# facebookresearch/rela

Measured on AMD Instinct MI355X. Metric: env-steps/s (Ape-X Atari 84x84x4, actor tick + learner grad-step), higher is better.
Workload: dtype f32 (f32 operands as 3 exact bf16 parts on bf16 MFMA; f32-accurate); 1 GPU; Ape-X DQN 80x80 envs/GPU, actor+learner on one MI355X, replay 2^20, B=512, A=18, n=3; device-resident static frames; parallelism=single

## Files before the change

rela_amd/csrc/gemm_s3.h:

```cpp
#pragma once
#include <hip/hip_runtime.h>

#include <algorithm>
#include <type_traits>

#include "common.h"
#include "gemm_f32emu.h"

namespace rela_amd {
namespace s3 {

using f32emu::bf16x2;
using f32emu::bf16x8;
using f32emu::f32x2;
using f32emu::f32x4;
using f32emu::kMaxBlocks;
using f32emu::kStageU4;
using f32emu::TN;
using f32emu::u32x4;
using f32emu::WRegs;

struct ProbConv2 {
  static constexpr int KS = 16, NCG = 1, OC = 64, PS = 64, REC = 192;
  __device__ static uint32_t row_base(int m) {
    const int n = m / 81, pos = m - n * 81;
    const int oy = pos / 9, ox = pos - oy * 9;
    return (uint32_t)(((n * 20 + 2 * oy) * 20 + 2 * ox) * REC);
  }
  __device__ static uint32_t koff(int ks) {
    const int tp = f32emu::ProbConv2::tap(ks);
    return (uint32_t)(((tp >> 2) * 20 + (tp & 3)) * REC);
  }
};
struct ProbConv3 {
  static constexpr int KS = 18, NCG = 1, OC = 64, PS = 128, REC = 384;
  __device__ static uint32_t row_base(int m) {
    const int n = m / 49, pos = m - n * 49;
    const int oy = pos / 7, ox = pos - oy * 7;
    return (uint32_t)(((n * 9 + oy) * 9 + ox) * REC);
  }
  __device__ static uint32_t koff(int ks) {
    const int tp = f32emu::ProbConv3::tap(ks);
    return (uint32_t)(((tp / 3) * 9 + tp % 3) * REC + (ks & 1) * 64);
  }
  __device__ static uint32_t pair_off(int kp) { return koff(2 * kp); }
};
template <int OC_>
struct ProbFcT {
  static constexpr int KS = 98, NCG = OC_ / 64, OC = OC_, PS = 128, REC = 384;
  __device__ static uint32_t row_base(int m) { return (uint32_t)m * (49u * REC); }
  __device__ static uint32_t koff(int ks) { return (uint32_t)((ks >> 1) * REC + (ks & 1) * 64); }
  __device__ static uint32_t pair_off(int kp) { return (uint32_t)(kp * REC); }
};
using ProbFc = ProbFcT<512>;

__device__ __forceinline__ void split3_4(const f32x4& v, uint2& p0, uint2& p1, uint2& p2) {
  const f32x2 a = {v[0], v[1]}, b = {v[2], v[3]};
  const bf16x2 a0 = __builtin_convertvector(a, bf16x2), b0 = __builtin_convertvector(b, bf16x2);
  const f32x2 ra = a - __builtin_convertvector(a0, f32x2), rb = b - __builtin_convertvector(b0, f32x2);
  const bf16x2 a1 = __builtin_convertvector(ra, bf16x2), b1 = __builtin_convertvector(rb, bf16x2);
  const f32x2 sa = ra - __builtin_convertvector(a1, f32x2), sb = rb - __builtin_convertvector(b1, f32x2);
  const bf16x2 a2 = __builtin_convertvector(sa, bf16x2), b2 = __builtin_convertvector(sb, bf16x2);
  p0 = make_uint2(__builtin_bit_cast(uint32_t, a0), __builtin_bit_cast(uint32_t, b0));
  p1 = make_uint2(__builtin_bit_cast(uint32_t, a1), __builtin_bit_cast(uint32_t, b1));
  p2 = make_uint2(__builtin_bit_cast(uint32_t, a2), __builtin_bit_cast(uint32_t, b2));
}

constexpr int kGemmT = 512;
constexpr int kGemmWaves = kGemmT / 64;
constexpr int kBlockCols = 128;
constexpr int TMV = 7;
constexpr int CT = 1;
static_assert(kGemmWaves * CT * 16 == kBlockCols, "the waves of a block tile its columns");
constexpr int kABuf = TMV * 6144;
constexpr int kBSlot = CT * 3072;
constexpr int kLdsB = 2 * kABuf;
constexpr int kLdsSpare = kLdsB + kGemmWaves * 2 * kBSlot;
constexpr int kLdsTotal = kLdsSpare + 1024;
static_assert(kLdsTotal <= 160 * 1024, "LDS budget");
__host__ __device__ constexpr int glds_per_wave(int nt) { return (6 * nt + kGemmWaves - 1) / kGemmWaves; }

typedef __attribute__((address_space(3))) uint8_t* lds_ptr_t;
typedef const __attribute__((address_space(1))) uint8_t* gbl_ptr_t;
__device__ __forceinline__ void glds16(const uint8_t* g, uint8_t* l) {
  __builtin_amdgcn_global_load_lds((gbl_ptr_t)g, (lds_ptr_t)l, 16, 0, 0);
}
#ifndef S3_GEMM_ABLATE
#define S3_GEMM_ABLATE 0
#endif
#ifndef S3_GEMM_AHEAD
#define S3_GEMM_AHEAD 1
#endif
constexpr int kAheadTiles = S3_GEMM_AHEAD;
template <int OFF>
__device__ __forceinline__ u32x4 lds_read128(uint32_t addr) {
  u32x4 r;
  asm volatile("ds_read_b128 %0, %1 offset:%2" : "=v"(r) : "v"(addr), "n"(OFF) : "memory");
  return r;
}
template <int N>
__device__ __forceinline__ void wait_lgkm(u32x4& a, u32x4& b, u32x4& c) {
  asm volatile("s_waitcnt lgkmcnt(%3)" : "+v"(a), "+v"(b), "+v"(c) : "n"(N) : "memory");
}
template <int N>
__device__ __forceinline__ void wait_vm() {
  asm volatile("s_waitcnt vmcnt(%0)" ::"n"(N) : "memory");
}
template <int I>
using IC = std::integral_constant<int, I>;
template <int N, class F>
__device__ __forceinline__ void static_for(F&& f) {
  if constexpr (N > 0) {
    static_for<N - 1>(f);
    f(IC<N - 1>{});
  }
}

struct Pipe {
  uint32_t g;
  uint32_t s;
};

template <class P>
__device__ __forceinline__ void issue_weights(const uint8_t* wsrc, uint8_t* lds, uint32_t bring, int k, uint32_t slot, uint32_t lane) {
  const uint8_t* src = wsrc + (size_t)k * (kStageU4 * 16) + lane * 16;
  uint8_t* dst = lds + bring + slot * kBSlot;
  if constexpr (S3_GEMM_ABLATE == 2) return;
#pragma unroll
  for (int q = 0; q < CT * 3; ++q) glds16(src + q * 1024, dst + q * 1024);
}

template <class P, int NT, int J>
__device__ __forceinline__ void k_pass(const uint8_t* __restrict__ Xb, const uint8_t* __restrict__ wsrc, uint8_t* lds, uint32_t lds0,
                                       const uint32_t (&offc)[J], const uint32_t (&offn)[J], const uint32_t (&ldst)[J],
                                       uint32_t frag_base, uint32_t wave, f32x4 (&acc)[NT][CT], f32x4 (&accs)[NT][CT], Pipe& pp,
                                       int kp0, int kp1) {
  constexpr int WL = 3 * CT;
  const uint32_t lane = threadIdx.x & 63;
  const uint32_t bring = kLdsB + wave * 2 * kBSlot;
  for (int kp = kp0; kp < kp1; ++kp) {
    const uint32_t abuf = (pp.g & 1) * kABuf;
    wait_vm<WL>();
    __builtin_amdgcn_s_barrier();
    {
      int k1 = 2 * kp + 1;
      issue_weights<P>(wsrc, lds, bring, k1, (pp.s + 1) & 1, lane);
      int k2 = kp + 1;
      const bool nextp = k2 >= kp1;
      if (nextp) k2 = kp0;
      const uint8_t* src = Xb + P::pair_off(k2);
      const uint32_t dst = ((pp.g + 1) & 1) * kABuf;
      if constexpr (S3_GEMM_ABLATE != 1) {
#pragma unroll
        for (int j = 0; j < J; ++j)
          glds16(src + (nextp ? offn[j] : offc[j]), lds + (ldst[j] >= (uint32_t)kLdsSpare ? ldst[j] : dst + ldst[j]));
      }
    }
    static_for<2>([&](auto hh) {
      constexpr int H = decltype(hh)::value;
      if constexpr (H == 1) {
        int k2 = 2 * kp + 2;
        if (k2 >= 2 * kp1) k2 = 2 * kp0;
        issue_weights<P>(wsrc, lds, bring, k2, (pp.s + 1) & 1, lane);
      }
      wait_vm<J + WL>();
      const uint32_t wa = lds0 + bring + (pp.s & 1) * kBSlot + lane * 16;
      u32x4 wq[CT][3];
      static_for<CT>([&](auto jj) {
        constexpr int JJ = decltype(jj)::value;
        wq[JJ][0] = lds_read128<JJ * 3072>(wa);
        wq[JJ][1] = lds_read128<JJ * 3072 + 1024>(wa);
        wq[JJ][2] = lds_read128<JJ * 3072 + 2048>(wa);
      });
      const uint32_t xa = lds0 + abuf + frag_base + H * 512;
      constexpr int RING = kAheadTiles + 1, PRE = NT < kAheadTiles ? NT : kAheadTiles;
      u32x4 x[RING][3];
      static_for<PRE>([&](auto tt) {
        constexpr int T = decltype(tt)::value;
        x[T][0] = lds_read128<T * 6144>(xa);
        x[T][1] = lds_read128<T * 6144 + 2048>(xa);
        x[T][2] = lds_read128<T * 6144 + 4096>(xa);
      });
      constexpr int AHEAD = PRE * 3;
      static_for<CT>([&](auto jj) {
        constexpr int JJ = decltype(jj)::value;
        wait_lgkm<AHEAD + 3 * (CT - 1 - JJ)>(wq[JJ][0], wq[JJ][1], wq[JJ][2]);
      });
      bf16x8 wf[CT][3];
#pragma unroll
      for (int j = 0; j < CT; ++j)
#pragma unroll
        for (int q = 0; q < 3; ++q) wf[j][q] = __builtin_bit_cast(bf16x8, wq[j][q]);
      static_for<NT>([&](auto tt) {
        constexpr int T = decltype(tt)::value;
        constexpr int C = T % RING;
        if constexpr (T + kAheadTiles < NT) {
          constexpr int N2 = (T + kAheadTiles) % RING;
          x[N2][0] = lds_read128<(T + kAheadTiles) * 6144>(xa);
          x[N2][1] = lds_read128<(T + kAheadTiles) * 6144 + 2048>(xa);
          x[N2][2] = lds_read128<(T + kAheadTiles) * 6144 + 4096>(xa);
        }
        constexpr int YOUNGER = 3 * ((T + kAheadTiles < NT ? T + kAheadTiles : NT - 1) - T);
        wait_lgkm<YOUNGER>(x[C][0], x[C][1], x[C][2]);
        const bf16x8 x0 = __builtin_bit_cast(bf16x8, x[C][0]), x1 = __builtin_bit_cast(bf16x8, x[C][1]),
                     x2 = __builtin_bit_cast(bf16x8, x[C][2]);
#pragma unroll
        for (int j = 0; j < CT; ++j) {
          accs[T][j] = __builtin_amdgcn_mfma_f32_16x16x32_bf16(wf[j][2], x0, accs[T][j], 0, 0, 0);
          accs[T][j] = __builtin_amdgcn_mfma_f32_16x16x32_bf16(wf[j][0], x2, accs[T][j], 0, 0, 0);
          accs[T][j] = __builtin_amdgcn_mfma_f32_16x16x32_bf16(wf[j][1], x1, accs[T][j], 0, 0, 0);
          accs[T][j] = __builtin_amdgcn_mfma_f32_16x16x32_bf16(wf[j][1], x0, accs[T][j], 0, 0, 0);
          accs[T][j] = __builtin_amdgcn_mfma_f32_16x16x32_bf16(wf[j][0], x1, accs[T][j], 0, 0, 0);
          acc[T][j] = __builtin_amdgcn_mfma_f32_16x16x32_bf16(wf[j][0], x0, acc[T][j], 0, 0, 0);
        }
        __builtin_amdgcn_sched_barrier(0);
      });
      pp.s += 1;
    });
    pp.g += 1;
  }
}

enum { kEpiRelu = 0, kEpiReluS3 = 1, kEpiRaw = 2, kEpiBias = 3 };
template <class P, int EPI>
__global__ __launch_bounds__(kGemmT, 1) void gemm_s3(const uint8_t* __restrict__ Xb, const uint4* __restrict__ Wp,
                                                 const float* __restrict__ bias, void* __restrict__ out_, int M) {
  constexpr int NCG = P::OC / kBlockCols;
  constexpr bool OUT_S3 = EPI == kEpiReluS3;
  const int kp0 = (int)((P::KS / 2) * blockIdx.y / gridDim.y), kp1 = (int)((P::KS / 2) * (blockIdx.y + 1) / gridDim.y);
  static_assert(P::OC % kBlockCols == 0, "a block owns 128 columns");
  __shared__ __attribute__((aligned(1024))) uint8_t lds[kLdsTotal];
  const uint32_t lds0 = (uint32_t)(size_t)(lds_ptr_t)lds;
  const int tid = threadIdx.x, lane = tid & 63, li = lane & 15, g = lane >> 4;
  const int wave = __builtin_amdgcn_readfirstlane(tid >> 6);
  const int xcd = blockIdx.x & 7, bi = blockIdx.x >> 3;
  const int cg = bi % NCG;
  const int rb = (bi / NCG) * 8 + xcd;
  const int nrb = gridDim.x / NCG;
  const int rt_total = (M + 15) >> 4;
  const int r0 = (int)((int64_t)rt_total * rb / nrb), r1 = (int)((int64_t)rt_total * (rb + 1) / nrb);
  const int cnt = r1 - r0;
  if (cnt <= 0) return;
  const int passes = (cnt + TMV - 1) / TMV;
  const int base = cnt / passes, rem = cnt - base * passes;
  const int ntmax = base + (rem ? 1 : 0);
  auto first_of = [&](int p) { return p < rem ? (base + 1) * p : (base + 1) * rem + base * (p - rem); };
  auto size_of = [&](int p) { return p < rem ? base + 1 : base; };
  const int cg64 = cg * 2 + (wave >> 2), u0 = wave & 3;
  const uint8_t* wsrc = reinterpret_cast<const uint8_t*>(Wp) + ((size_t)cg64 * P::KS * kStageU4 + (size_t)u0 * 3 * 64) * 16;
  const int col0 = cg * kBlockCols + 16 * CT * wave + 4 * g;
  const uint32_t frag_base = (uint32_t)((li >> 3) * 1024 + (16 * (g >> 1) + 2 * (li & 7) + (g & 1)) * 16);
  const int lr = (lane & 15) >> 1, lu = 2 * (lane >> 4) + (lane & 1);

  f32x4 bv[CT];
#pragma unroll
  for (int j = 0; j < CT; ++j) {
    if constexpr (EPI == kEpiRaw)
      bv[j] = f32x4{0.f, 0.f, 0.f, 0.f};
    else
      bv[j] = *reinterpret_cast<const f32x4*>(bias + col0 + 16 * j);
    asm volatile("" : "+v"(bv[j]));
  }
  Pipe pp{0u, 0u};

  auto run = [&](auto ntm) {
    constexpr int NTM = decltype(ntm)::value, J = glds_per_wave(NTM);
    uint32_t offc[J], offn[J], ldst[J];
    auto set_off = [&](uint32_t (&off)[J], int p) {
      const int nt = size_of(p), t0 = r0 + first_of(p);
#pragma unroll
      for (int j = 0; j < J; ++j) {
        int i = wave + kGemmWaves * j;
        if (i >= 6 * nt) i = 0;
        const int part = (i >> 1) % 3, t = i / 6, b = i & 1;
        const int row = min((t0 + t) * 16 + b * 8 + lr, M - 1);
        off[j] = P::row_base(row) + (uint32_t)(part * 128 + lu * 16);
      }
    };
#pragma unroll
    for (int j = 0; j < J; ++j) {
      const int i = wave + kGemmWaves * j;
      ldst[j] = i < 6 * ntmax ? (uint32_t)i * 1024u : (uint32_t)kLdsSpare;
    }
    set_off(offc, 0);
    set_off(offn, min(1, passes - 1));
    {
      const uint8_t* src = Xb + P::pair_off(kp0);
#pragma unroll
      for (int j = 0; j < J; ++j) glds16(src + offc[j], lds + ldst[j]);
      issue_weights<P>(wsrc, lds, kLdsB + wave * 2 * kBSlot, 2 * kp0, 0, lane);
    }
    auto one_pass = [&](auto ntag, int p) {
      constexpr int NT = decltype(ntag)::value;
      f32x4 acc[NT][CT], accs[NT][CT];
#pragma unroll
      for (int t = 0; t < NT; ++t)
#pragma unroll
        for (int j = 0; j < CT; ++j) acc[t][j] = bv[j], accs[t][j] = f32x4{0.f, 0.f, 0.f, 0.f};
      k_pass<P, NT, J>(Xb, wsrc, lds, lds0, offc, offn, ldst, frag_base, wave, acc, accs, pp, kp0, kp1);
      const int t0 = r0 + first_of(p);
#pragma unroll
      for (int t = 0; t < NT; ++t) {
        const int row = (t0 + t) * 16 + li;
        if (row < M) {
#pragma unroll
          for (int j = 0; j < CT; ++j) {
            f32x4 v = acc[t][j] + accs[t][j];
            if constexpr (EPI == kEpiRelu || EPI == kEpiReluS3) {
#pragma unroll
              for (int r = 0; r < 4; ++r) v[r] = v[r] > 0.f ? v[r] : 0.f;
            }
            if constexpr (OUT_S3) {
              uint8_t* o = reinterpret_cast<uint8_t*>(out_) + (size_t)row * (6 * P::OC) + (col0 + 16 * j) * 2;
              uint2 p0, p1, p2;
              split3_4(v, p0, p1, p2);
              *reinterpret_cast<uint2*>(o) = p0;
              *reinterpret_cast<uint2*>(o + 2 * P::OC) = p1;
              *reinterpret_cast<uint2*>(o + 4 * P::OC) = p2;
            } else {
              *reinterpret_cast<f32x4*>(reinterpret_cast<float*>(out_) + ((size_t)blockIdx.y * M + row) * P::OC + col0 + 16 * j) = v;
            }
          }
        }
      }
    };
    for (int p = 0; p < passes; ++p) {
      if (size_of(p) == NTM)
        one_pass(IC<NTM>{}, p);
      else if constexpr (NTM > 1)
        one_pass(IC<NTM - 1>{}, p);
#pragma unroll
      for (int j = 0; j < J; ++j) offc[j] = offn[j];
      set_off(offn, min(p + 2, passes - 1));
    }
  };
  switch (ntmax) {
    case 1: run(IC<1>{}); break;
    case 2: run(IC<2>{}); break;
    case 3: run(IC<3>{}); break;
    case 4: run(IC<4>{}); break;
    case 5: run(IC<5>{}); break;
    case 6: run(IC<6>{}); break;
    default: run(IC<7>{}); break;
  }
  wait_vm<0>();
}

struct Plan {
  int nrb, slices;
};
template <class P>
inline Plan plan(int M, bool may_split) {
  constexpr int NCG = P::OC / kBlockCols;
  const int rt_total = (M + 15) / 16;
  const int full = kMaxBlocks / 2;
  Plan pl;
  pl.nrb = (std::min(full / NCG, rt_total) + 7) / 8 * 8;
  pl.slices = 1;
  if (may_split && pl.nrb * NCG * 4 <= full * 3) {
    pl.nrb = ((rt_total + 3) / 4 + 7) / 8 * 8;
    pl.slices = std::max(1, std::min(8, full / (pl.nrb * NCG)));
  }
  return pl;
}
template <class P, int EPI>
inline void launch(const void* X, const uint4* Wp, const float* bias, void* out, int M, hipStream_t s, Plan pl) {
  constexpr int NCG = P::OC / kBlockCols;
  hipLaunchKernelGGL((gemm_s3<P, EPI>), dim3(pl.nrb * NCG, EPI == kEpiRaw ? pl.slices : 1), dim3(kGemmT), 0, s,
                     reinterpret_cast<const uint8_t*>(X), Wp, bias, out, M);
}
template <class P, int EPI>
inline void launch(const void* X, const uint4* Wp, const float* bias, void* out, int M, hipStream_t s) {
  launch<P, EPI>(X, Wp, bias, out, M, s, plan<P>(M, false));
}

template <int C>
__global__ void split_s3(const float* __restrict__ x, uint8_t* __restrict__ rec, int64_t pixels) {
  const int64_t i = (int64_t)blockIdx.x * blockDim.x + threadIdx.x;
  if (i >= pixels * (C / 4)) return;
  const int64_t px = i / (C / 4);
  const int c4 = (int)(i - px * (C / 4));
  const f32x4 v = *reinterpret_cast<const f32x4*>(x + px * C + c4 * 4);
  uint2 p0, p1, p2;
  split3_4(v, p0, p1, p2);
  uint8_t* o = rec + px * (6 * C) + c4 * 8;
  *reinterpret_cast<uint2*>(o) = p0;
  *reinterpret_cast<uint2*>(o + 2 * C) = p1;
  *reinterpret_cast<uint2*>(o + 4 * C) = p2;
}
template <int C>
__global__ void unsplit_s3(const uint8_t* __restrict__ rec, float* __restrict__ x, int64_t pixels) {
  const int64_t i = (int64_t)blockIdx.x * blockDim.x + threadIdx.x;
  if (i >= pixels * (C / 4)) return;
  const int64_t px = i / (C / 4);
  const int c4 = (int)(i - px * (C / 4));
  const uint8_t* r = rec + px * (6 * C) + c4 * 8;
  const uint2 p0 = *reinterpret_cast<const uint2*>(r), p1 = *reinterpret_cast<const uint2*>(r + 2 * C),
              p2 = *reinterpret_cast<const uint2*>(r + 4 * C);
  auto f = [](uint32_t w, int hi) { return __builtin_bit_cast(float, hi ? (w & 0xffff0000u) : (w << 16)); };
  f32x4 v;
  v[0] = (f(p0.x, 0) + f(p1.x, 0)) + f(p2.x, 0);
  v[1] = (f(p0.x, 1) + f(p1.x, 1)) + f(p2.x, 1);
  v[2] = (f(p0.y, 0) + f(p1.y, 0)) + f(p2.y, 0);
  v[3] = (f(p0.y, 1) + f(p1.y, 1)) + f(p2.y, 1);
  *reinterpret_cast<f32x4*>(x + px * C + c4 * 4) = v;
}

}
}
```

Before: 3.694 million env-steps/s.

## Interleave LDS-DMA issues across MFMA slots via compile-time pair schedule

```diff
diff --git a/rela_amd/csrc/gemm_s3.h b/rela_amd/csrc/gemm_s3.h
--- a/rela_amd/csrc/gemm_s3.h
+++ b/rela_amd/csrc/gemm_s3.h
@@ -130,40 +130,98 @@
   for (int q = 0; q < CT * 3; ++q) glds16(src + q * 1024, dst + q * 1024);
 }
 
-template <class P, int NT, int J>
+#ifndef S3_GEMM_PLACE
+#define S3_GEMM_PLACE 0
+#endif
+#ifndef S3_GEMM_PLACE_HI
+#define S3_GEMM_PLACE_HI S3_GEMM_PLACE
+#endif
+#ifndef S3_GEMM_PRIO
+#define S3_GEMM_PRIO 0
+#endif
+constexpr int kMaxGldsRun = 2;
+template <int NT, int J, int PL>
+struct PairSched {
+  static constexpr int JA = S3_GEMM_ABLATE == 1 ? 0 : J;
+  static constexpr int WL = S3_GEMM_ABLATE == 2 ? 0 : 3 * CT;
+  static constexpr int N = JA + 2 * WL;
+  static constexpr int SUB = N > 2 * NT ? 2 : 1;
+  static constexpr int S = 2 * NT * SUB;
+  static constexpr int CAP = N > S ? (N + S - 1) / S : 1;
+  static constexpr int pos(int i) {
+    int p = PL == 0 ? i / CAP : PL == 1 ? i * S / N : S - 1 - (N - 1 - i) / CAP;
+    if (i >= JA + WL) {
+      const int lo = S / 2 + (i - JA - WL) / CAP;
+      if (p < lo) p = lo;
+    }
+    return p;
+  }
+  static constexpr int count_at(int p) {
+    int c = 0;
+    for (int i = 0; i < N; ++i) c += pos(i) == p;
+    return c;
+  }
+  static constexpr int first_half() {
+    int c = 0;
+    for (int i = 0; i < N; ++i) c += pos(i) < S / 2;
+    return c;
+  }
+  static constexpr bool valid() {
+    for (int i = 0; i < N; ++i) {
+      if (pos(i) < 0 || pos(i) >= S) return false;
+      if (i && pos(i) < pos(i - 1)) return false;
+      if (i >= JA + WL && pos(i) < S / 2) return false;
+    }
+    for (int p = 0; p < S; ++p)
+      if (count_at(p) > kMaxGldsRun) return false;
+    if (S3_GEMM_ABLATE == 0 && first_half() == 0) return false;
+    return true;
+  }
+  static_assert(valid(), "the pair's LDS-DMA schedule");
+};
+
+template <class P, int NT, int J, int PL>
 __device__ __forceinline__ void k_pass(const uint8_t* __restrict__ Xb, const uint8_t* __restrict__ wsrc, uint8_t* lds, uint32_t lds0,
                                        const uint32_t (&offc)[J], const uint32_t (&offn)[J], const uint32_t (&ldst)[J],
                                        uint32_t frag_base, uint32_t wave, f32x4 (&acc)[NT][CT], f32x4 (&accs)[NT][CT], Pipe& pp,
                                        int kp0, int kp1) {
-  constexpr int WL = 3 * CT;
+  using SC = PairSched<NT, J, PL>;
+  static_assert(CT == 1, "the positions of PairSched are those of one column tile's MFMAs");
   const uint32_t lane = threadIdx.x & 63;
   const uint32_t bring = kLdsB + wave * 2 * kBSlot;
   for (int kp = kp0; kp < kp1; ++kp) {
     const uint32_t abuf = (pp.g & 1) * kABuf;
-    wait_vm<WL>();
+    wait_vm<2 * SC::WL>();
     __builtin_amdgcn_s_barrier();
-    {
-      int k1 = 2 * kp + 1;
-      issue_weights<P>(wsrc, lds, bring, k1, (pp.s + 1) & 1, lane);
-      int k2 = kp + 1;
-      const bool nextp = k2 >= kp1;
-      if (nextp) k2 = kp0;
-      const uint8_t* src = Xb + P::pair_off(k2);
-      const uint32_t dst = ((pp.g + 1) & 1) * kABuf;
-      if constexpr (S3_GEMM_ABLATE != 1) {
-#pragma unroll
-        for (int j = 0; j < J; ++j)
-          glds16(src + (nextp ? offn[j] : offc[j]), lds + (ldst[j] >= (uint32_t)kLdsSpare ? ldst[j] : dst + ldst[j]));
+    int k2 = kp + 1;
+    const bool nextp = k2 >= kp1;
+    if (nextp) k2 = kp0;
+    const uint8_t* asrc = Xb + P::pair_off(k2);
+    const uint32_t adst = ((pp.g + 1) & 1) * kABuf;
+    const uint8_t* wsrc2 = wsrc + (size_t)(2 * k2) * (kStageU4 * 16) + lane * 16;
+    uint8_t* const wdst0 = lds + bring + (pp.s & 1) * kBSlot;
+    uint8_t* const wdst1 = lds + bring + ((pp.s + 1) & 1) * kBSlot;
+    auto issue_at = [&](auto pt) {
+      constexpr int PT = decltype(pt)::value;
+      if constexpr (SC::count_at(PT) > 0) {
+        static_for<SC::N>([&](auto ii) {
+          constexpr int I = decltype(ii)::value;
+          if constexpr (SC::pos(I) == PT) {
+            if constexpr (I < SC::JA) {
+              glds16(asrc + (nextp ? offn[I] : offc[I]), lds + (ldst[I] >= (uint32_t)kLdsSpare ? ldst[I] : adst + ldst[I]));
+            } else if constexpr (I < SC::JA + SC::WL) {
+              glds16(wsrc2 + (I - SC::JA) * 1024, wdst0 + (I - SC::JA) * 1024);
+            } else {
+              glds16(wsrc2 + kStageU4 * 16 + (I - SC::JA - SC::WL) * 1024, wdst1 + (I - SC::JA - SC::WL) * 1024);
+            }
+          }
+        });
+        __builtin_amdgcn_sched_barrier(0);
       }
-    }
+    };
     static_for<2>([&](auto hh) {
       constexpr int H = decltype(hh)::value;
-      if constexpr (H == 1) {
-        int k2 = 2 * kp + 2;
-        if (k2 >= 2 * kp1) k2 = 2 * kp0;
-        issue_weights<P>(wsrc, lds, bring, k2, (pp.s + 1) & 1, lane);
-      }
-      wait_vm<J + WL>();
+      wait_vm<H == 0 ? SC::WL : SC::first_half()>();
       const uint32_t wa = lds0 + bring + (pp.s & 1) * kBSlot + lane * 16;
       u32x4 wq[CT][3];
       static_for<CT>([&](auto jj) {
@@ -204,16 +262,18 @@
         wait_lgkm<YOUNGER>(x[C][0], x[C][1], x[C][2]);
         const bf16x8 x0 = __builtin_bit_cast(bf16x8, x[C][0]), x1 = __builtin_bit_cast(bf16x8, x[C][1]),
                      x2 = __builtin_bit_cast(bf16x8, x[C][2]);
-#pragma unroll
-        for (int j = 0; j < CT; ++j) {
-          accs[T][j] = __builtin_amdgcn_mfma_f32_16x16x32_bf16(wf[j][2], x0, accs[T][j], 0, 0, 0);
-          accs[T][j] = __builtin_amdgcn_mfma_f32_16x16x32_bf16(wf[j][0], x2, accs[T][j], 0, 0, 0);
-          accs[T][j] = __builtin_amdgcn_mfma_f32_16x16x32_bf16(wf[j][1], x1, accs[T][j], 0, 0, 0);
-          accs[T][j] = __builtin_amdgcn_mfma_f32_16x16x32_bf16(wf[j][1], x0, accs[T][j], 0, 0, 0);
-          accs[T][j] = __builtin_amdgcn_mfma_f32_16x16x32_bf16(wf[j][0], x1, accs[T][j], 0, 0, 0);
-          acc[T][j] = __builtin_amdgcn_mfma_f32_16x16x32_bf16(wf[j][0], x0, acc[T][j], 0, 0, 0);
+        accs[T][0] = __builtin_amdgcn_mfma_f32_16x16x32_bf16(wf[0][2], x0, accs[T][0], 0, 0, 0);
+        accs[T][0] = __builtin_amdgcn_mfma_f32_16x16x32_bf16(wf[0][0], x2, accs[T][0], 0, 0, 0);
+        accs[T][0] = __builtin_amdgcn_mfma_f32_16x16x32_bf16(wf[0][1], x1, accs[T][0], 0, 0, 0);
+        if constexpr (SC::SUB == 2) {
+          if constexpr (SC::count_at((H * NT + T) * 2) > 0) __builtin_amdgcn_sched_barrier(0);
+          issue_at(IC<(H * NT + T) * 2>{});
         }
+        accs[T][0] = __builtin_amdgcn_mfma_f32_16x16x32_bf16(wf[0][1], x0, accs[T][0], 0, 0, 0);
+        accs[T][0] = __builtin_amdgcn_mfma_f32_16x16x32_bf16(wf[0][0], x1, accs[T][0], 0, 0, 0);
+        acc[T][0] = __builtin_amdgcn_mfma_f32_16x16x32_bf16(wf[0][0], x0, acc[T][0], 0, 0, 0);
         __builtin_amdgcn_sched_barrier(0);
+        issue_at(IC<(H * NT + T) * SC::SUB + SC::SUB - 1>{});
       });
       pp.s += 1;
     });
@@ -262,8 +322,11 @@
     asm volatile("" : "+v"(bv[j]));
   }
   Pipe pp{0u, 0u};
-
-  auto run = [&](auto ntm) {
+  if constexpr (S3_GEMM_PRIO == 1) {
+    if (wave >= 4) __builtin_amdgcn_s_setprio(1);
+  }
+
+  auto run =[&](auto ntm) {
     constexpr int NTM = decltype(ntm)::value, J = glds_per_wave(NTM);
     uint32_t offc[J], offn[J], ldst[J];
     auto set_off = [&](uint32_t (&off)[J], int p) {
@@ -289,6 +352,7 @@
 #pragma unroll
       for (int j = 0; j < J; ++j) glds16(src + offc[j], lds + ldst[j]);
       issue_weights<P>(wsrc, lds, kLdsB + wave * 2 * kBSlot, 2 * kp0, 0, lane);
+      issue_weights<P>(wsrc, lds, kLdsB + wave * 2 * kBSlot, 2 * kp0 + 1, 1, lane);
     }
     auto one_pass = [&](auto ntag, int p) {
       constexpr int NT = decltype(ntag)::value;
@@ -297,7 +361,14 @@
       for (int t = 0; t < NT; ++t)
 #pragma unroll
         for (int j = 0; j < CT; ++j) acc[t][j] = bv[j], accs[t][j] = f32x4{0.f, 0.f, 0.f, 0.f};
-      k_pass<P, NT, J>(Xb, wsrc, lds, lds0, offc, offn, ldst, frag_base, wave, acc, accs, pp, kp0, kp1);
+      if constexpr (S3_GEMM_PLACE_HI != S3_GEMM_PLACE) {
+        if (wave >= 4)
+          k_pass<P, NT, J, S3_GEMM_PLACE_HI>(Xb, wsrc, lds, lds0, offc, offn, ldst, frag_base, wave, acc, accs, pp, kp0, kp1);
+        else
+          k_pass<P, NT, J, S3_GEMM_PLACE>(Xb, wsrc, lds, lds0, offc, offn, ldst, frag_base, wave, acc, accs, pp, kp0, kp1);
+      } else {
+        k_pass<P, NT, J, S3_GEMM_PLACE>(Xb, wsrc, lds, lds0, offc, offn, ldst, frag_base, wave, acc, accs, pp, kp0, kp1);
+      }
       const int t0 = r0 + first_of(p);
 #pragma unroll
       for (int t = 0; t < NT; ++t) {
```

Result: faster. 3.746 million env-steps/s, median of 6 (+1.4%).
